# lyclyc52/Segment-Anything-NeRF

Measured on AMD Instinct MI355X. Metric: rays/sec (RGB+256-d SAM feat) at 512×512, 1/2/4/8 MI355X; PSNR vs ref, higher is better.
Workload: dtype fp32-equivalent: fp32 in the reference's op order for everything that decides a discrete result (near/far, bins, proposal grids + MLPs, compositing, sample_pdf); grid_mlp (32->64->64->16 per sample), the SAM head (163->256x5) and the mask head (143->256->256->K per sample) as f16x3: each fp32 produc

## Files before the change

### segment-anything-nerf_amd/csrc/sam_head.hip

```cpp
#include "samnerf_common.h"
#include "f16x3.h"

namespace samnerf {

namespace {

constexpr int kRows = 32;
constexpr int kXPad = 168;
constexpr int kXStride = 169;
constexpr int kHStride = 257;
constexpr int kIn = 163;
constexpr int kRowIn = 164;
constexpr int kK[5] = {kXPad, 256, 256 + kXPad, 256, 256};
constexpr int kGroups[5] = {kXPad / 8, 256 / 8, (256 + kXPad) / 8, 256 / 8, 256 / 8};
constexpr int kLogicalIn[5] = {kIn, 256, 256 + kIn, 256, 256};

__host__ __device__ constexpr int group_base(int layer) {
    int b = 0;
    for (int i = 0; i < layer; ++i) b += kGroups[i];
    return b;
}
constexpr int kTotalGroups = group_base(5);

__device__ __forceinline__ int logical_k(int layer, int kp) {
// ... 596 lines not shown
    const char* rows;
    const char* rows_end;
    uint32_t xs;
    uint32_t next_tile;
    int wave, lane;
    int rot;
    int step;

    __device__ __forceinline__ int buf(int s) const {
        const int b = rot + s % NBUF;
        return b >= NBUF ? b - NBUF : b;
    }
    __device__ __forceinline__ void wpiece(int s, int c) {
        const uint4* base = packed + (size_t)(s % kSteps) * kStepVec + (size_t)wave * 256 + (size_t)c * 64;
        lds_dma16(base + lane, (uint32_t)reinterpret_cast<uintptr_t>(Wb + buf(s) * kStepVec + wave * 256 + c * 64));
    }
    __device__ __forceinline__ void xpiece(int q) {
        const uint32_t p = (uint32_t)(wave * kXPieces + q);
        const char* base = rows + (size_t)next_tile * kTileBytes + (size_t)p * 1024u;
        const char* src = base + (size_t)lane * 16u;
        src = src > rows_end ? rows_end : src;
        lds_dma16(src, xs + p * 1024u);
    }
    static __device__ __forceinline__ constexpr bool xstep(int s) { return s >= kXFirst && s < kXFirst + kXPieces; }

    __device__ __forceinline__ void run(floatx16 (&acc)[8], const uint4& bh, const uint4& bl) {
        const int s = step;
        const uint4* cur = Wb + buf(s) * kStepVec + lane;
        uint4 fh[8], fl[8];
#pragma unroll
        for (int t = 0; t < 8; ++t) {
            fh[t] = cur[t * 64];
            fl[t] = cur[512 + t * 64];
        }
#pragma unroll
        for (int t = 0; t < 8; ++t) {
            acc[t] = mfma_f16x3(fh[t], fl[t], bh, bl, acc[t]);
            if (t & 1) {
                __builtin_amdgcn_sched_barrier(0);
                wpiece(s + NBUF - 1, t >> 1);
                __builtin_amdgcn_sched_barrier(0);
            }
        }
        if (xstep(s)) {
            __builtin_amdgcn_sched_barrier(0);
            xpiece(s - kXFirst);
            __builtin_amdgcn_sched_barrier(0);
        }
        int n = 4 * (NBUF - 2);
#pragma unroll
        for (int k = s + 2 - NBUF; k <= s; ++k) n += xstep(k) ? 1 : 0;
        wait_vmn(n);
        asm volatile("s_waitcnt lgkmcnt(0)" ::: "memory");
        __builtin_amdgcn_s_barrier();
        ++step;
    }
};

template <int NBUF, bool STAMP = false, bool VEC = true>
__global__ void __launch_bounds__(256) __attribute__((amdgpu_waves_per_eu(1, 1)))
k_sam_head_h16q(HeadArgsH a, uint32_t ntiles) {
    unsigned long long t0 = 0, rt0 = 0;
    if constexpr (STAMP) {
        t0 = __builtin_amdgcn_s_memtime();
        rt0 = __builtin_amdgcn_s_memrealtime();
    }
    __shared__ uint4 smem[NBUF * kStepVec + kXVec + (7 * 256 + 8) / 4];
    uint4* const Wb = smem;
    float* const Xs = reinterpret_cast<float*>(smem + NBUF * kStepVec);
    float* const Bs = reinterpret_cast<float*>(smem + NBUF * kStepVec + kXVec);
    const int tid = threadIdx.x, wave = tid >> 6, lane = tid & 63;
    const int j = lane & 31, h = lane >> 5;

    for (int i = tid; i < 5 * 256; i += 256) Bs[i] = a.b[i >> 8][i & 255];
    float* const Wi = Bs + 7 * 256;
    if (tid < 5) Wi[tid] = exp2i(-a.kexp[tid]);
    Bs[5 * 256 + tid] = a.ln_w[tid];
    Bs[6 * 256 + tid] = a.ln_b[tid];

    HeadStreamQ<NBUF> st;
    st.packed = a.packed + (size_t)((blockIdx.x >> 3) % kHeadCopies) * kPackedVec;
    st.Wb = Wb;
    st.rows = reinterpret_cast<const char*>(a.rows);
    st.rows_end = st.rows + (size_t)a.N * kRowIn * 4 - 16;
    st.xs = (uint32_t)reinterpret_cast<uintptr_t>(Xs);
    st.next_tile = blockIdx.x;
    st.wave = __builtin_amdgcn_readfirstlane(wave);
    st.lane = lane;
    st.rot = 0;
    st.step = 0;
#pragma unroll
    for (int q = 0; q < kXPieces; ++q) st.xpiece(q);
#pragma unroll
    for (int q = 0; q + 1 < NBUF; ++q)
#pragma unroll
        for (int c = 0; c < 4; ++c) st.wpiece(q, c);
    wait_vmn(4 * (NBUF - 2));
    asm volatile("s_waitcnt lgkmcnt(0)" ::: "memory");
    __syncthreads();

    const float* xr = Xs + (wave * 32 + j) * kRowIn;
    for (uint32_t tile = blockIdx.x; tile < ntiles; tile += gridDim.x) {
        st.next_tile = tile + gridDim.x;
        st.step = 0;
        asm volatile("" : "+s"(st.packed), "+s"(st.rows));
        const uint32_t ray = tile * kRaysV5 + wave * 32u + j;
        const bool live = ray < a.N;
        auto x8 = [&](int kb, float (&v)[8]) {
            const int c0 = 16 * kb + 8 * h;
            if (c0 + 8 <= kRowIn) {
                const float4 p = *reinterpret_cast<const float4*>(xr + c0);
                const float4 q = *reinterpret_cast<const float4*>(xr + c0 + 4);
                v[0] = p.x; v[1] = p.y; v[2] = p.z; v[3] = p.w;
                v[4] = q.x; v[5] = q.y; v[6] = q.z; v[7] = q.w;
            } else {
#pragma unroll
                for (int m = 0; m < 8; ++m) v[m] = c0 + m < kRowIn ? xr[c0 + m] : 0.0f;
            }
#pragma unroll
            for (int m = 0; m < 8; ++m)
                if (!live || c0 + m >= kIn) v[m] = 0.0f;
        };
        float xmax = 0.0f;
#pragma unroll
        for (int kb = 0; kb < kXkb; ++kb) {
            float v[8];
            x8(kb, v);
#pragma unroll
            for (int m = 0; m < 8; ++m) xmax = fmaxf(xmax, fabsf(v[m]));
        }
        xmax = fmaxf(xmax, __shfl_xor(xmax, 32));
        auto load_x = [&](float sc_s, uint4 (&xh)[kXkb], uint4 (&xl)[kXkb]) {
#pragma unroll
            for (int kb = 0; kb < kXkb; ++kb) {
                float v[8];
                x8(kb, v);
                split8_f16(v, sc_s, xh[kb], xl[kb]);
            }
        };
        uint4 xh[kXkb], xl[kXkb];
        Scale2 sc = scale_of_max(xmax);
        load_x(sc.s, xh, xl);

        floatx16 acc[8];
        uint4 ah[kHkb], al[kHkb];
        auto zero = [&]() {
#pragma unroll
            for (int t = 0; t < 8; ++t) acc[t] = floatx16{};
        };
        auto next = [&](int layer, float extra) {
            float m = finish_layer(acc, Bs + layer * 256, sc.inv * Wi[layer], h, true);
            m = fmaxf(fmaxf(m, __shfl_xor(m, 32)), extra);
            sc = scale_of_max(m);
            split_layer(acc, sc.s, ah, al);
        };
        auto h_segment = [&]() {
#pragma unroll
            for (int kb = 0; kb < kHkb; ++kb) st.run(acc, ah[kb], al[kb]);
        };

        zero();
#pragma unroll
        for (int kb = 0; kb < kXkb; ++kb) st.run(acc, xh[kb], xl[kb]);
        next(0, 0.0f);
        zero();
        h_segment();
        next(1, xmax);
        zero();
        load_x(sc.s, xh, xl);
#pragma unroll
        for (int kb = 0; kb < kXkb; ++kb) st.run(acc, xh[kb], xl[kb]);
        h_segment();
        next(2, 0.0f);
        zero();
        h_segment();
        next(3, 0.0f);
        zero();
        h_segment();
        finish_layer(acc, Bs + 4 * 256, sc.inv * Wi[4], h, false);

        double s = 0.0;
#pragma unroll
        for (int t = 0; t < 8; ++t)
#pragma unroll
            for (int q = 0; q < 16; ++q) s += (double)acc[t][q];
        s += __shfl_xor(s, 32);
        const double mean = s / 256.0;
        double var = 0.0;
#pragma unroll
        for (int t = 0; t < 8; ++t)
#pragma unroll
            for (int q = 0; q < 16; ++q) {
                const double dlt = (double)acc[t][q] - mean;
                var += dlt * dlt;
            }
        var += __shfl_xor(var, 32);
        const float rstd = (float)(1.0 / sqrt(var / 256.0 + 1e-5));
        const float mf = (float)mean;
        if (live) {
            float* o = a.out + (size_t)ray * a.ld;
            const float* lw = Bs + 5 * 256;
            const float* lb = Bs + 6 * 256;
#pragma unroll
            for (int t = 0; t < 8; ++t)
#pragma unroll
                for (int mm = 0; mm < 4; ++mm) {
                    const int u = 32 * t + 8 * mm + 4 * h;
                    float4 y;
                    y.x = ((acc[t][4 * mm + 0] - mf) * rstd) * lw[u + 0] + lb[u + 0];
                    y.y = ((acc[t][4 * mm + 1] - mf) * rstd) * lw[u + 1] + lb[u + 1];
                    y.z = ((acc[t][4 * mm + 2] - mf) * rstd) * lw[u + 2] + lb[u + 2];
                    y.w = ((acc[t][4 * mm + 3] - mf) * rstd) * lw[u + 3] + lb[u + 3];
                    store_out4(o + u, y, VEC);
                }
        }
        st.rot = (st.rot + kSteps) % NBUF;
    }
    wait_vmn(0);
    if constexpr (STAMP) {
        const unsigned long long t1 = __builtin_amdgcn_s_memtime(), rt1 = __builtin_amdgcn_s_memrealtime();
        if (lane == 0) {
            unsigned long long* o = a.stamps + ((size_t)blockIdx.x * 4 + wave) * 16;
            for (int i = 0; i < 16; ++i) o[i] = 0;
            o[12] = t1 - t0;
            o[13] = rt1 - rt0;
        }
    }
}

#ifndef SAMNERF_HEAD_W8
#define SAMNERF_HEAD_W8 1
#endif
#if defined(SAMNERF_DIAG_VARIANTS) || SAMNERF_HEAD_W8
namespace w8 {
constexpr int kXkb = 6;
constexpr int kHkb = 8;
constexpr int kSegKb[6] = {kXkb, kHkb, kXkb, kHkb, kHkb, kHkb};
constexpr int kSegLayer[6] = {0, 1, 2, 2, 3, 4};
constexpr int segBase(int seg) {
    int b = 0;
    for (int i = 0; i < seg; ++i) b += kSegKb[i];
    return b;
}
constexpr int kKb = segBase(6);
constexpr int kSteps = 2 * kKb;
constexpr int kStepVec = 2 * 8 * 64;
constexpr int kPackedVec = kSteps * kStepVec;
constexpr int kRays = 16;
constexpr int kWaves = 8;
constexpr int kXPieces = 11;
constexpr int kXRegion = 84;
constexpr int kXFirst = 30;
static_assert(kXPieces * kWaves * 1024 >= kTileBytes, "x pieces cover a tile");
static_assert(kXRegion * 1024 >= kTileBytes && kXRegion * 1024 <= kXVec * 16, "x region");
static_assert(kXFirst > 2 * (kXkb + kHkb) + 1 && kXFirst + kXPieces + 3 < kSteps, "x stream window");

__host__ __device__ constexpr int hunit(int b, int g, int m) { return 32 * b + (m < 4 ? 4 * g + m : 16 + 4 * g + m - 4); }

__device__ __forceinline__ float weight(const float* const* W, int kb, int unit, int g, int m) {
    int seg = 0;
    while (seg < 5 && kb >= segBase(seg + 1)) ++seg;
    const int b = kb - segBase(seg);
    const int kx = 32 * b + 8 * g + m;
    switch (seg) {
        case 0: return kx < kIn ? W[0][unit * kIn + kx] : 0.0f;
        case 1: return W[1][unit * 256 + hunit(b, g, m)];
        case 2: return kx < kIn ? W[2][unit * (256 + kIn) + 256 + kx] : 0.0f;
        case 3: return W[2][unit * (256 + kIn) + hunit(b, g, m)];
        case 4: return W[3][unit * 256 + hunit(b, g, m)];
        default: return W[4][unit * 256 + hunit(b, g, m)];
    }
}
}

__global__ void __launch_bounds__(256) k_pack_w8(PackArgs a) {
    __shared__ int kx;
    const uint32_t t = blockIdx.x * blockDim.x + threadIdx.x;
    const int bstep = (int)((blockIdx.x * blockDim.x) >> 9);
    int bseg = 0;
    while (bseg < 5 && (bstep >> 1) >= w8::segBase(bseg + 1)) ++bseg;
    const int layer = w8::kSegLayer[bseg];
    if (threadIdx.x < 64) {
        float m = threadIdx.x < kWmaxParts ? a.part[layer * kWmaxParts + threadIdx.x] : 0.0f;
        m = wave_max64(m);
        if (threadIdx.x == 0) {
            kx = scale_exp_of_max(m);
            a.kexp[layer] = kx;
        }
    }
    __syncthreads();
    if (t >= (uint32_t)w8::kSteps * 8u * 64u) return;
    const int lane = (int)(t & 63u), tile = (int)((t >> 6) & 7u), step = (int)(t >> 9);
    const int kb = step >> 1, unit = 16 * (8 * (step & 1) + tile) + (lane & 15), g = lane >> 4;
    float v[8];
#pragma unroll
    for (int e = 0; e < 8; ++e) v[e] = w8::weight(a.W, kb, unit, g, e);
    uint4 hi, lo;
    split8_f16(v, exp2i(kx), hi, lo);
    a.packed[(size_t)step * w8::kStepVec + tile * 64 + lane] = hi;
    a.packed[(size_t)step * w8::kStepVec + 512 + tile * 64 + lane] = lo;
}


template <int NBUF, int WAVES>
struct HeadStreamW8 {
    static constexpr int kPieces = 16 / WAVES;
    const uint4* packed;
    uint4* Wb;
    const char* rows;
    const char* rows_end;
    uint32_t xs;
    uint32_t sink;
    uint32_t next_tile;
    int wave, lane;
    int rot;
    int step;

    __device__ __forceinline__ int buf(int s) const {
        const int b = rot + s % NBUF;
        return b >= NBUF ? b - NBUF : b;
    }
    __device__ __forceinline__ void wpiece(int s, int c) {
        const int o = wave * 64 * kPieces + c * 64;
        const uint4* base = packed + (size_t)(s % w8::kSteps) * w8::kStepVec + (size_t)o;
        lds_dma16(base + lane, (uint32_t)reinterpret_cast<uintptr_t>(Wb + buf(s) * w8::kStepVec + o));
    }
    __device__ __forceinline__ void xpiece(int q) {
        const uint32_t p = (uint32_t)(wave * w8::kXPieces + q);
        const char* src = rows + (size_t)next_tile * kTileBytes + (size_t)p * 1024u + (size_t)lane * 16u;
        src = src > rows_end ? rows_end : src;
        lds_dma16(src, p < (uint32_t)w8::kXRegion ? xs + p * 1024u : sink);
    }
    static __device__ __forceinline__ constexpr bool xstep(int s) {
        return WAVES == 8 && s >= w8::kXFirst && s < w8::kXFirst + w8::kXPieces;
    }

    template <int HALF>
    __device__ __forceinline__ void run(floatx4 (&acc)[16], const uint4& bh, const uint4& bl) {
        const int s = step;
        const uint4* cur = Wb + buf(s) * w8::kStepVec + lane;
        uint4 fh[8], fl[8];
#pragma unroll
        for (int t = 0; t < 8; ++t) {
            fh[t] = cur[t * 64];
            fl[t] = cur[512 + t * 64];
        }
#pragma unroll
        for (int t = 0; t < 8; ++t) {
            acc[8 * HALF + t] = mfma16_f16x3(fh[t], fl[t], bh, bl, acc[8 * HALF + t]);
            if (t % (8 / kPieces) == 8 / kPieces - 1) {
                __builtin_amdgcn_sched_barrier(0);
                wpiece(s + NBUF - 1, t / (8 / kPieces));
                __builtin_amdgcn_sched_barrier(0);
            }
        }
        if (xstep(s)) {
            __builtin_amdgcn_sched_barrier(0);
            xpiece(s - w8::kXFirst);
            __builtin_amdgcn_sched_barrier(0);
        }
        int n = kPieces * (NBUF - 2);
#pragma unroll
        for (int k = s + 2 - NBUF; k <= s; ++k) n += xstep(k) ? 1 : 0;
        wait_vmn(n);
        asm volatile("s_waitcnt lgkmcnt(0)" ::: "memory");
        __builtin_amdgcn_s_barrier();
        ++step;
    }
};

__device__ __forceinline__ float finish_w8(floatx4 (&acc)[16], const float* Bs, float inv, int g, bool act) {
    float m = 0.0f;
#pragma unroll
    for (int t = 0; t < 16; ++t) {
        const float4 bb = *reinterpret_cast<const float4*>(Bs + 16 * t + 4 * g);
        const float b4[4] = {bb.x, bb.y, bb.z, bb.w};
#pragma unroll
        for (int r = 0; r < 4; ++r) acc[t][r] = leaky(__builtin_fmaf(acc[t][r], inv, b4[r]), act);
        m = max_abs3(m, acc[t][0], acc[t][1]);
        m = max_abs3(m, acc[t][2], acc[t][3]);
    }
    return m;
}

__device__ __forceinline__ void split_w8(const floatx4 (&acc)[16], float s, uint4 (&ah)[w8::kHkb],
                                         uint4 (&al)[w8::kHkb]) {
#pragma unroll
    for (int b = 0; b < w8::kHkb; ++b) {
        const float v[8] = {acc[2 * b][0], acc[2 * b][1], acc[2 * b][2], acc[2 * b][3],
                            acc[2 * b + 1][0], acc[2 * b + 1][1], acc[2 * b + 1][2], acc[2 * b + 1][3]};
        split8_f16<true>(v, s, ah[b], al[b]);
    }
}

__device__ __forceinline__ float ray_max4(float m) {
    m = fmaxf(m, __shfl_xor(m, 16));
    return fmaxf(m, __shfl_xor(m, 32));
}
__device__ __forceinline__ double ray_sum4(double v) {
    v += __shfl_xor(v, 16);
    return v + __shfl_xor(v, 32);
}

constexpr int kW8SinkVec = 64;

template <int NBUF, int WAVES, bool VEC = true>
__global__ void __launch_bounds__(64 * WAVES) __attribute__((amdgpu_waves_per_eu(2, 2)))
k_sam_head_w8(HeadArgsH a, uint32_t ntiles) {
    constexpr bool XLDS = WAVES == 8;
    constexpr int kTileRays = WAVES * w8::kRays;
    constexpr int kX = XLDS ? kXVec + kW8SinkVec : 0;
    __shared__ uint4 smem[NBUF * w8::kStepVec + kX + (7 * 256 + 8) / 4];
    uint4* const Wb = smem;
    float* const Xs = reinterpret_cast<float*>(smem + NBUF * w8::kStepVec);
    float* const Bs = reinterpret_cast<float*>(smem + NBUF * w8::kStepVec + kX);
    const int tid = threadIdx.x, wave = tid >> 6, lane = tid & 63;
    const int j = lane & 15, g = lane >> 4;
    if (XLDS && wave >= 4) __builtin_amdgcn_s_setprio(1);

    for (int i = tid; i < 5 * 256; i += 64 * WAVES) Bs[i] = a.b[i >> 8][i & 255];
    float* const Wi = Bs + 7 * 256;
    if (tid < 5) Wi[tid] = exp2i(-a.kexp[tid]);
    if (tid < 256) {
        Bs[5 * 256 + tid] = a.ln_w[tid];
        Bs[6 * 256 + tid] = a.ln_b[tid];
    }

    HeadStreamW8<NBUF, WAVES> st;
    st.packed = a.packed;
    st.Wb = Wb;
    st.rows = reinterpret_cast<const char*>(a.rows);
    st.rows_end = st.rows + (size_t)a.N * kRowIn * 4 - 16;
    st.xs = (uint32_t)reinterpret_cast<uintptr_t>(Xs);
    st.sink = (uint32_t)reinterpret_cast<uintptr_t>(smem + NBUF * w8::kStepVec + kXVec);
    st.next_tile = blockIdx.x;
    st.wave = __builtin_amdgcn_readfirstlane(wave);
    st.lane = lane;
    st.rot = 0;
    st.step = 0;
    if constexpr (XLDS) {
#pragma unroll
        for (int q = 0; q < w8::kXPieces; ++q) st.xpiece(q);
    }
#pragma unroll
    for (int q = 0; q + 1 < NBUF; ++q)
#pragma unroll
        for (int c = 0; c < st.kPieces; ++c) st.wpiece(q, c);
    wait_vmn(st.kPieces * (NBUF - 2));
    asm volatile("s_waitcnt lgkmcnt(0)" ::: "memory");
    __syncthreads();

    for (uint32_t tile = blockIdx.x; tile < ntiles; tile += gridDim.x) {
        st.next_tile = tile + gridDim.x;
        st.step = 0;
        asm volatile("" : "+s"(st.packed), "+s"(st.rows));
        const uint32_t ray = tile * kTileRays + wave * w8::kRays + j;
        const bool live = ray < a.N;
        const float* xr = XLDS ? Xs + (wave * w8::kRays + j) * kRowIn : a.rows + (size_t)(live ? ray : 0u) * kRowIn;
        auto x8 = [&](int kb, float (&v)[8]) {
            const int c0 = 32 * kb + 8 * g;
            if (c0 + 8 <= kRowIn) {
                const float4 p = *reinterpret_cast<const float4*>(xr + c0);
                const float4 q = *reinterpret_cast<const float4*>(xr + c0 + 4);
                v[0] = p.x; v[1] = p.y; v[2] = p.z; v[3] = p.w;
                v[4] = q.x; v[5] = q.y; v[6] = q.z; v[7] = q.w;
            } else {
#pragma unroll
                for (int m = 0; m < 8; ++m) v[m] = c0 + m < kRowIn ? xr[c0 + m] : 0.0f;
            }
#pragma unroll
            for (int m = 0; m < 8; ++m)
                if (!live || c0 + m >= kIn) v[m] = 0.0f;
        };
        float xmax = 0.0f;
#pragma unroll
        for (int kb = 0; kb < w8::kXkb; ++kb) {
            float v[8];
            x8(kb, v);
#pragma unroll
            for (int m = 0; m < 8; ++m) xmax = fmaxf(xmax, fabsf(v[m]));
        }
        xmax = ray_max4(xmax);
        uint4 xh[w8::kXkb], xl[w8::kXkb];
        auto load_x = [&](float sc_s) {
#pragma unroll
            for (int kb = 0; kb < w8::kXkb; ++kb) {
                float v[8];
                x8(kb, v);
                split8_f16<true>(v, sc_s, xh[kb], xl[kb]);
            }
        };
        Scale2 sc = scale_of_max(xmax);
        load_x(sc.s);

        floatx4 acc[16];
        uint4 ah[w8::kHkb], al[w8::kHkb];
        auto zero = [&]() {
#pragma unroll
            for (int t = 0; t < 16; ++t) acc[t] = floatx4{};
        };
        auto next = [&](int layer, float extra) {
            float m = finish_w8(acc, Bs + layer * 256, sc.inv * Wi[layer], g, true);
            m = fmaxf(ray_max4(m), extra);
            sc = scale_of_max(m);
            split_w8(acc, sc.s, ah, al);
        };
        auto x_segment = [&]() {
#pragma unroll
            for (int kb = 0; kb < w8::kXkb; ++kb) {
                st.template run<0>(acc, xh[kb], xl[kb]);
                st.template run<1>(acc, xh[kb], xl[kb]);
            }
        };
        auto h_segment = [&]() {
#pragma unroll
            for (int kb = 0; kb < w8::kHkb; ++kb) {
                st.template run<0>(acc, ah[kb], al[kb]);
                st.template run<1>(acc, ah[kb], al[kb]);
            }
        };

        zero();
        x_segment();
        next(0, 0.0f);
        zero();
        h_segment();
        next(1, xmax);
        zero();
        load_x(sc.s);
        x_segment();
        h_segment();
        next(2, 0.0f);
        zero();
        h_segment();
        next(3, 0.0f);
        zero();
        h_segment();
        finish_w8(acc, Bs + 4 * 256, sc.inv * Wi[4], g, false);

        double s = 0.0;
#pragma unroll
        for (int t = 0; t < 16; ++t)
#pragma unroll
            for (int r = 0; r < 4; ++r) s += (double)acc[t][r];
        s = ray_sum4(s);
        const double mean = s / 256.0;
        double var = 0.0;
#pragma unroll
        for (int t = 0; t < 16; ++t)
#pragma unroll
            for (int r = 0; r < 4; ++r) {
                const double dlt = (double)acc[t][r] - mean;
                var += dlt * dlt;
            }
        var = ray_sum4(var);
        const float rstd = (float)(1.0 / sqrt(var / 256.0 + 1e-5));
        const float mf = (float)mean;
        if (live) {
            float* o = a.out + (size_t)ray * a.ld;
            const float* lw = Bs + 5 * 256;
            const float* lb = Bs + 6 * 256;
#pragma unroll
            for (int t = 0; t < 16; ++t) {
                const int u = 16 * t + 4 * g;
                float4 y;
                y.x = ((acc[t][0] - mf) * rstd) * lw[u + 0] + lb[u + 0];
                y.y = ((acc[t][1] - mf) * rstd) * lw[u + 1] + lb[u + 1];
                y.z = ((acc[t][2] - mf) * rstd) * lw[u + 2] + lb[u + 2];
                y.w = ((acc[t][3] - mf) * rstd) * lw[u + 3] + lb[u + 3];
                store_out4(o + u, y, VEC);
            }
        }
        st.rot = (st.rot + w8::kSteps) % NBUF;
    }
    wait_vmn(0);
}
#endif

#ifdef SAMNERF_DIAG_VARIANTS
template <int TPW>
struct PairCfg {
    static constexpr int WPG = 8 / TPW;
    static constexpr int NW = 4 * WPG;
    static constexpr int NT = 64 * NW;
    static constexpr int PIECES = 16 / NW;
};
constexpr int kBVec = kHkb * 2 * 64;
constexpr int kPairSmemVec = 2 * kStepVec + 4 * kBVec;

__device__ __forceinline__ void lds_barrier() {
    asm volatile("s_waitcnt lgkmcnt(0)" ::: "memory");
    __builtin_amdgcn_s_barrier();
    asm volatile("" ::: "memory");
}

template <int TPW>
__global__ void __launch_bounds__(PairCfg<TPW>::NT)
__attribute__((amdgpu_waves_per_eu(PairCfg<TPW>::WPG, PairCfg<TPW>::WPG)))
k_sam_head_h16p(HeadArgsH a) {
    using C = PairCfg<TPW>;
    __shared__ uint4 smem[kPairSmemVec];
    uint4* const Wb = smem;
    const int tid = threadIdx.x, wave = tid >> 6, lane = tid & 63;
    const int grp = wave / C::WPG, part = wave % C::WPG;
    const int t0 = part * TPW;
    uint4* const Bg = smem + 2 * kStepVec + grp * kBVec;
    const int j = lane & 31, h = lane >> 5;
    const uint32_t ray = blockIdx.x * kRaysV5 + grp * 32u + j;
    const bool live = ray < a.N;
    const float* xr = a.rows + (size_t)(live ? ray : 0u) * kRowIn;

    auto issue = [&](int s) {
        const uint4* src = a.packed + (size_t)s * kStepVec + wave * (64 * C::PIECES) + lane;
        const uint32_t dst = (uint32_t)reinterpret_cast<uintptr_t>(Wb + (s & 1) * kStepVec + wave * (64 * C::PIECES));
#pragma unroll
        for (int c = 0; c < C::PIECES; ++c) lds_dma16(src + c * 64, dst + c * 1024u);
    };
    auto xload = [&](int kb, float4& p, float4& q) {
        if (kb < kXkb - 1) {
            p = *reinterpret_cast<const float4*>(xr + 16 * kb + 8 * h);
            q = *reinterpret_cast<const float4*>(xr + 16 * kb + 8 * h + 4);
        } else {
            p = *reinterpret_cast<const float4*>(xr + 160);
            q = p;
        }
    };
    auto xvals = [&](int kb, const float4& p, const float4& q, float (&v)[8]) {
        v[0] = p.x; v[1] = p.y; v[2] = p.z; v[3] = p.w;
        v[4] = q.x; v[5] = q.y; v[6] = q.z; v[7] = q.w;
        const int c0 = 16 * kb + 8 * h;
#pragma unroll
        for (int m = 0; m < 8; ++m)
            if (!live || c0 + m >= kIn) v[m] = 0.0f;
    };

    int s = 0;
    issue(0);
    float xmax = 0.0f;
#pragma unroll
    for (int kb = 0; kb < kXkb; ++kb) {
        float4 p, q;
        float v[8];
        xload(kb, p, q);
        xvals(kb, p, q, v);
#pragma unroll
        for (int m = 0; m < 8; ++m) xmax = fmaxf(xmax, fabsf(v[m]));
    }
    xmax = fmaxf(xmax, __shfl_xor(xmax, 32));
    float Wi[5];
#pragma unroll
    for (int l = 0; l < 5; ++l) Wi[l] = exp2i(-a.kexp[l]);
    Scale2 sc = scale_of_max(xmax);
    asm volatile("s_waitcnt vmcnt(0)" ::: "memory");
    lds_barrier();

    floatx16 acc[TPW];
    auto zero = [&]() {
#pragma unroll
        for (int t = 0; t < TPW; ++t) acc[t] = floatx16{};
    };
    auto mma = [&](const uint4& bh, const uint4& bl) {
        const uint4* cur = Wb + (s & 1) * kStepVec + lane;
        uint4 fh[TPW], fl[TPW];
#pragma unroll
        for (int t = 0; t < TPW; ++t) {
            fh[t] = cur[(t0 + t) * 64];
            fl[t] = cur[512 + (t0 + t) * 64];
        }
#pragma unroll
        for (int t = 0; t < TPW; ++t) acc[t] = mfma_f16x3(fh[t], fl[t], bh, bl, acc[t]);
        asm volatile("s_waitcnt vmcnt(0)" ::: "memory");
        lds_barrier();
        ++s;
    };
    auto x_segment = [&]() {
        float4 p, q;
        xload(0, p, q);
#pragma unroll
        for (int kb = 0; kb < kXkb; ++kb) {
            float v[8];
            xvals(kb, p, q, v);
            uint4 bh, bl;
            split8_f16(v, sc.s, bh, bl);
            if (s + 1 < kSteps) issue(s + 1);
            if (kb + 1 < kXkb) xload(kb + 1, p, q);
            mma(bh, bl);
        }
    };
    auto h_segment = [&]() {
#pragma unroll
        for (int kb = 0; kb < kHkb; ++kb) {
            const uint4 bh = Bg[(2 * kb) * 64 + lane], bl = Bg[(2 * kb + 1) * 64 + lane];
            if (s + 1 < kSteps) issue(s + 1);
            mma(bh, bl);
        }
    };
    auto next = [&](int layer, float extra) {
        const float inv = sc.inv * Wi[layer];
        const float* bias = a.b[layer];
        float m = 0.0f;
#pragma unroll
        for (int t = 0; t < TPW; ++t)
#pragma unroll
            for (int mm = 0; mm < 4; ++mm) {
                const float4 bb = *reinterpret_cast<const float4*>(bias + 32 * (t0 + t) + 8 * mm + 4 * h);
                const float b4[4] = {bb.x, bb.y, bb.z, bb.w};
#pragma unroll
                for (int e = 0; e < 4; ++e)
                    acc[t][4 * mm + e] = leaky(__builtin_fmaf(acc[t][4 * mm + e], inv, b4[e]), true);
#pragma unroll
                for (int e = 0; e < 4; e += 2) m = max_abs3(m, acc[t][4 * mm + e], acc[t][4 * mm + e + 1]);
            }
        m = fmaxf(m, __shfl_xor(m, 32));
        float* X = reinterpret_cast<float*>(Wb + ((s + 1) & 1) * kStepVec);
        if (h == 0) X[(grp * C::WPG + part) * 32 + j] = m;
        lds_barrier();
        float mm2 = 0.0f;
#pragma unroll
        for (int p = 0; p < C::WPG; ++p) mm2 = fmaxf(mm2, X[(grp * C::WPG + p) * 32 + j]);
        sc = scale_of_max(fmaxf(mm2, extra));
#pragma unroll
        for (int t = 0; t < TPW; ++t) {
            float v[16];
#pragma unroll
            for (int q = 0; q < 16; ++q) v[q] = acc[t][q];
            uint4 hi, lo;
            split8_f16(v, sc.s, hi, lo);
            Bg[(2 * (2 * (t0 + t))) * 64 + lane] = hi;
            Bg[(2 * (2 * (t0 + t)) + 1) * 64 + lane] = lo;
            split8_f16(v + 8, sc.s, hi, lo);
            Bg[(2 * (2 * (t0 + t) + 1)) * 64 + lane] = hi;
            Bg[(2 * (2 * (t0 + t) + 1) + 1) * 64 + lane] = lo;
        }
        lds_barrier();
    };

    zero();
    x_segment();
    next(0, 0.0f);
    zero();
    h_segment();
    next(1, xmax);
    zero();
    x_segment();
    h_segment();
    next(2, 0.0f);
    zero();
    h_segment();
    next(3, 0.0f);
    zero();
    h_segment();

    float4* Y = reinterpret_cast<float4*>(Bg);
    {
        const float inv = sc.inv * Wi[4];
        const float* bias = a.b[4];
#pragma unroll
        for (int t = 0; t < TPW; ++t)
#pragma unroll
            for (int mm = 0; mm < 4; ++mm) {
                const float4 bb = *reinterpret_cast<const float4*>(bias + 32 * (t0 + t) + 8 * mm + 4 * h);
                float4 y;
                y.x = __builtin_fmaf(acc[t][4 * mm + 0], inv, bb.x);
                y.y = __builtin_fmaf(acc[t][4 * mm + 1], inv, bb.y);
                y.z = __builtin_fmaf(acc[t][4 * mm + 2], inv, bb.z);
                y.w = __builtin_fmaf(acc[t][4 * mm + 3], inv, bb.w);
                Y[((t0 + t) * 4 + mm) * 64 + lane] = y;
            }
    }
    lds_barrier();
    double sum = 0.0;
#pragma unroll
    for (int t = 0; t < 8; ++t) {
#pragma unroll
        for (int mm = 0; mm < 4; ++mm) {
            const float4 y = Y[(t * 4 + mm) * 64 + lane];
            sum += (double)y.x;
            sum += (double)y.y;
            sum += (double)y.z;
            sum += (double)y.w;
        }
        asm volatile("" ::: "memory");
    }
    sum += __shfl_xor(sum, 32);
    const double mean = sum / 256.0;
    double var = 0.0;
#pragma unroll
    for (int t = 0; t < 8; ++t) {
#pragma unroll
        for (int mm = 0; mm < 4; ++mm) {
            const float4 y = Y[(t * 4 + mm) * 64 + lane];
            const float yy[4] = {y.x, y.y, y.z, y.w};
#pragma unroll
            for (int e = 0; e < 4; ++e) {
                const double dlt = (double)yy[e] - mean;
                var += dlt * dlt;
            }
        }
        asm volatile("" ::: "memory");
    }
    var += __shfl_xor(var, 32);
    const float rstd = (float)(1.0 / sqrt(var / 256.0 + 1e-5));
    const float mf = (float)mean;
    if (!live) return;
    float* o = a.out + (size_t)ray * a.ld;
#pragma unroll
    for (int t = 0; t < TPW; ++t)
#pragma unroll
        for (int mm = 0; mm < 4; ++mm) {
            const int u = 32 * (t0 + t) + 8 * mm + 4 * h;
            const float4 v = Y[((t0 + t) * 4 + mm) * 64 + lane];
            const float4 lw = *reinterpret_cast<const float4*>(a.ln_w + u);
            const float4 lb = *reinterpret_cast<const float4*>(a.ln_b + u);
            float4 y;
            y.x = ((v.x - mf) * rstd) * lw.x + lb.x;
            y.y = ((v.y - mf) * rstd) * lw.y + lb.y;
            y.z = ((v.z - mf) * rstd) * lw.z + lb.z;
            y.w = ((v.w - mf) * rstd) * lw.w + lb.w;
            store_out4(o + u, y, a.vec_out);
        }
}

#endif

}

static int device_cus() {
    static int cus[64] = {0};
    int dev = 0;
    if (hipGetDevice(&dev) != hipSuccess || dev < 0 || dev >= 64) return 256;
    if (!cus[dev]) {
        int n = 0;
        if (hipDeviceGetAttribute(&n, hipDeviceAttributeMultiprocessorCount, dev) != hipSuccess || n <= 0) n = 256;
        cus[dev] = n;
    }
    return cus[dev];
}

[[maybe_unused]] static int head_w8() {
#ifdef SAMNERF_DIAG_VARIANTS
    const char* v = diag_env("SAMNERF_HEAD_V");
    if (v) return atoi(v) == 30 ? 1 : atoi(v) == 31 ? 2 : 0;
#endif
    return SAMNERF_HEAD_W8;
}

size_t sam_head_packed_floats() {
    const size_t f32 = (size_t)8 * kTotalGroups * 64 * 4;
    const size_t h16 = (size_t)kPackedVec * 4 * kHeadCopies + 8 + 5 * kWmaxParts;
    const size_t hw8 = (size_t)88 * 1024 * 4 + 8 + 5 * kWmaxParts;
    const size_t m = f32 > h16 ? f32 : h16;
    return m > hw8 ? m : hw8;
}

int sam_head_forward(const samnerf_model* m, const float* rows, uint32_t N, float* samvit,
                     float* packed, hipStream_t s, uint32_t ld, bool pack) {
    const bool vec = ld % 4u == 0u && reinterpret_cast<uintptr_t>(samvit) % 16u == 0u;
#if defined(SAMNERF_DIAG_VARIANTS) || SAMNERF_HEAD_W8
    if (m->head_mode == 0 && head_w8()) {
        PackArgs p;
        for (int i = 0; i < 5; ++i) p.W[i] = m->sam_w[i];
        p.packed = reinterpret_cast<uint4*>(packed);
        p.kexp = reinterpret_cast<int*>(packed + (size_t)w8::kPackedVec * 4);
        p.part = packed + (size_t)w8::kPackedVec * 4 + 8;
        if (pack) {
            k_head_wmax<<<dim3(kWmaxParts, 5), 256, 0, s>>>(p);
            k_pack_w8<<<div_up((uint32_t)w8::kSteps * 8u * 64u, 256), 256, 0, s>>>(p);
        }
        HeadArgsH a{};
        a.rows = rows;
        a.N = N;
        a.packed = p.packed;
        a.kexp = p.kexp;
        for (int i = 0; i < 5; ++i) a.b[i] = m->sam_b[i];
        a.ln_w = m->ln_w;
        a.ln_b = m->ln_b;
        a.out = samvit;
        a.ld = ld;
        a.vec_out = vec;
        if (head_w8() == 2) {
            const uint32_t blocks = div_up(N, 64u);
            const uint32_t grid = blocks < 2u * (uint32_t)device_cus() ? blocks : 2u * (uint32_t)device_cus();
            if (vec) k_sam_head_w8<4, 4><<<grid, 256, 0, s>>>(a, blocks);
            else k_sam_head_w8<4, 4, false><<<grid, 256, 0, s>>>(a, blocks);
        } else {
            const uint32_t blocks = div_up(N, (uint32_t)kRaysV5);
            const uint32_t grid = blocks < (uint32_t)device_cus() ? blocks : (uint32_t)device_cus();
            if (vec) k_sam_head_w8<4, 8><<<grid, 512, 0, s>>>(a, blocks);
            else k_sam_head_w8<4, 8, false><<<grid, 512, 0, s>>>(a, blocks);
        }
        return check_launch("sam_head_w8");
    }
#endif
    if (m->head_mode == 0) {
        PackArgs p;
        for (int i = 0; i < 5; ++i) p.W[i] = m->sam_w[i];
        p.packed = reinterpret_cast<uint4*>(packed);
        p.kexp = reinterpret_cast<int*>(packed + (size_t)kPackedVec * 4 * kHeadCopies);
        p.part = packed + (size_t)kPackedVec * 4 * kHeadCopies + 8;
        if (pack) {
            k_head_wmax<<<dim3(kWmaxParts, 5), 256, 0, s>>>(p);
            k_pack_h16<<<div_up((uint32_t)kSteps * 8u * 64u, 256), 256, 0, s>>>(p);
        }
        HeadArgsH a;
        a.rows = rows;
        a.N = N;
        a.packed = p.packed;
        a.kexp = p.kexp;
        for (int i = 0; i < 5; ++i) a.b[i] = m->sam_b[i];
        a.ln_w = m->ln_w;
        a.ln_b = m->ln_b;
        a.out = samvit;
        a.ld = ld;
        a.vec_out = vec;
        a.stamps = nullptr;
        const uint32_t blocks = div_up(N, (uint32_t)kRaysV5);
#ifdef SAMNERF_DIAG_VARIANTS
        const char* v = diag_env("SAMNERF_HEAD_V");
        const int form = v ? atoi(v) : 0;
        const uint32_t grid = blocks < (uint32_t)device_cus() ? blocks : (uint32_t)device_cus();
        if (form == 20) k_sam_head_h16q<3><<<grid, 256, 0, s>>>(a, blocks);
        else if (form == 21 || form == 13) {
            const char* p = diag_env("SAMNERF_HEAD_STAMPS");
            a.stamps = reinterpret_cast<unsigned long long*>(p ? strtoull(p, nullptr, 16) : 0ull);
            if (!a.stamps) return fail(SAMNERF_EINVAL, "sam_head form %d needs SAMNERF_HEAD_STAMPS", form);
            if (form == 21) k_sam_head_h16q<4, true><<<grid, 256, 0, s>>>(a, blocks);
            else k_sam_head_h16<3, true, 1, false, true><<<blocks, 256, 0, s>>>(a);
        }
        else if (form == 1) k_sam_head_h16<3, false, 1><<<blocks, 256, 0, s>>>(a);
        else if (form == 2) k_sam_head_h16p<4><<<blocks, PairCfg<4>::NT, 0, s>>>(a);
        else if (form == 3) k_sam_head_h16p<2><<<blocks, PairCfg<2>::NT, 0, s>>>(a);
        else if (form == 5) k_sam_head_h16<3, false, 2><<<blocks, 256, 0, s>>>(a);
        else if (form == 6) k_sam_head_h16<4, true, 1><<<blocks, 256, 0, s>>>(a);
        else if (form == 7) k_sam_head_h16<3, true, 2><<<blocks, 256, 0, s>>>(a);
        else if (form == 8) k_sam_head_h16<4, true, 2><<<blocks, 256, 0, s>>>(a);
        else if (form == 11) k_sam_head_h16<3, true, 0><<<blocks, 256, 0, s>>>(a);
        else if (form == 12) k_sam_head_h16<3, true, 1, true><<<blocks, 256, 0, s>>>(a);
        else if (form == 4) k_sam_head_h16<3, true, 1><<<blocks, 256, 0, s>>>(a);
        else
#endif
        {
            const uint32_t grid = blocks < (uint32_t)device_cus() ? blocks : (uint32_t)device_cus();
            if (vec) k_sam_head_h16q<4><<<grid, 256, 0, s>>>(a, blocks);
            else k_sam_head_h16q<4, false, false><<<grid, 256, 0, s>>>(a, blocks);
        }
        return check_launch("sam_head_h16");
    }
    const uint32_t nvec = 8u * kTotalGroups * 64u;
    if (pack)
        k_pack<<<div_up(nvec, 256), 256, 0, s>>>(m->sam_w[0], m->sam_w[1], m->sam_w[2], m->sam_w[3],
                                                 m->sam_w[4], packed);
    HeadArgs a;
    a.rows = rows;
    a.N = N;
    a.packed = packed;
    for (int i = 0; i < 5; ++i) a.b[i] = m->sam_b[i];
    a.ln_w = m->ln_w;
    a.ln_b = m->ln_b;
    a.out = samvit;
    a.ld = ld;
    a.vec_out = vec;
    k_sam_head<<<div_up(N, kRows), 256, 0, s>>>(a);
    return check_launch("sam_head");
}

}

extern "C" {

size_t samnerf_sam_head_workspace_size(void) { return samnerf::sam_head_packed_floats() * sizeof(float); }

int samnerf_sam_head_forward(const samnerf_model* m, const float* rows, uint32_t N, float* samvit,
                             void* workspace, size_t workspace_bytes, samnerf_stream_t stream) {
    using namespace samnerf;
    if (!m) return fail(SAMNERF_EINVAL, "sam_head_forward: null model");
    if (!m->with_sam) return fail(SAMNERF_EINVAL, "sam_head_forward: model has no SAM head (with_sam = 0)");
    for (int i = 0; i < 5; ++i)
        if (!m->sam_w[i] || !m->sam_b[i]) return fail(SAMNERF_EINVAL, "sam_head_forward: null head weight");
    if (!m->ln_w || !m->ln_b) return fail(SAMNERF_EINVAL, "sam_head_forward: null LayerNorm weight");
    if (m->head_mode != 0 && m->head_mode != 1)
        return fail(SAMNERF_EINVAL, "sam_head_forward: head_mode must be 0 or 1, got %d", m->head_mode);
    if (N == 0) return SAMNERF_OK;
    if (!rows || !samvit || !workspace) return fail(SAMNERF_EINVAL, "sam_head_forward: null pointer");
    const size_t need = samnerf_sam_head_workspace_size();
    if (workspace_bytes < need)
        return fail(SAMNERF_EWORKSPACE, "sam_head_forward: workspace needs %zu bytes, got %zu", need,
                    workspace_bytes);
    return sam_head_forward(m, rows, N, samvit, static_cast<float*>(workspace),
                            reinterpret_cast<hipStream_t>(stream), 256u, true);
}

}
```

Before: 98.29 million.

## Software-pipeline LDS weight fragment loads across steps in the W8 SAM head

Adds a pipelined loop for the 8-wave W8 SAM head kernel. Half of the next step's weight fragments are read from LDS before the barrier while the current MFMAs run, and the DMA of the next weight piece now runs one step further ahead using all NBUF buffers. The default path now uses the pipelined variant with both pieces issued at the last MFMA (PLACE=1). It also adds diagnostic variants with timestamp probes, and an output-address tweak that uses mbcnt for the lane group. The aim is to hide LDS read latency and barrier stalls behind MFMA work, at the cost of more register pressure from holding fragments in the struct and tighter buffer reuse.

```diff
diff --git a/segment-anything-nerf_amd/csrc/sam_head.hip b/segment-anything-nerf_amd/csrc/sam_head.hip
--- a/segment-anything-nerf_amd/csrc/sam_head.hip
+++ b/segment-anything-nerf_amd/csrc/sam_head.hip
@@ -922,9 +922,12 @@
 }
 
 
-template <int NBUF, int WAVES>
+template <int NBUF, int WAVES, bool PIPE = false, bool STAMP = false, int PLACE = 0>
 struct HeadStreamW8 {
     static constexpr int kPieces = 16 / WAVES;
+    static constexpr int kAhead = PIPE ? NBUF : NBUF - 1;
+    uint4 fh[8], fl[8];
+    unsigned long long ts[4];
     const uint4* packed;
     uint4* Wb;
     const char* rows;
@@ -940,8 +943,10 @@
         const int b = rot + s % NBUF;
         return b >= NBUF ? b - NBUF : b;
     }
+    static constexpr bool kLowMoves = PLACE == 2;
+    __device__ __forceinline__ bool mover() const { return !kLowMoves || wave < 4; }
     __device__ __forceinline__ void wpiece(int s, int c) {
-        const int o = wave * 64 * kPieces + c * 64;
+        const int o = wave * 64 * (kLowMoves ? 4 : kPieces) + c * 64;
         const uint4* base = packed + (size_t)(s % w8::kSteps) * w8::kStepVec + (size_t)o;
         lds_dma16(base + lane, (uint32_t)reinterpret_cast<uintptr_t>(Wb + buf(s) * w8::kStepVec + o));
     }
@@ -955,16 +960,28 @@
         return WAVES == 8 && s >= w8::kXFirst && s < w8::kXFirst + w8::kXPieces;
     }
 
+    static __device__ __forceinline__ unsigned long long now() {
+        unsigned long long t = __builtin_amdgcn_s_memtime();
+        asm volatile("s_waitcnt lgkmcnt(0)" : "+s"(t)::"memory");
+        return t;
+    }
+
     template <int HALF>
     __device__ __forceinline__ void run(floatx4 (&acc)[16], const uint4& bh, const uint4& bl) {
+        if constexpr (PIPE) {
+            run_pipe<HALF>(acc, bh, bl);
+            return;
+        }
         const int s = step;
         const uint4* cur = Wb + buf(s) * w8::kStepVec + lane;
-        uint4 fh[8], fl[8];
+        unsigned long long t0 = 0, t1 = 0, t2 = 0;
+        if constexpr (STAMP) t0 = now();
 #pragma unroll
         for (int t = 0; t < 8; ++t) {
             fh[t] = cur[t * 64];
             fl[t] = cur[512 + t * 64];
         }
+        if constexpr (STAMP) t1 = now();
 #pragma unroll
         for (int t = 0; t < 8; ++t) {
             acc[8 * HALF + t] = mfma16_f16x3(fh[t], fl[t], bh, bl, acc[8 * HALF + t]);
@@ -979,13 +996,94 @@
             xpiece(s - w8::kXFirst);
             __builtin_amdgcn_sched_barrier(0);
         }
+        if constexpr (STAMP) t2 = now();
         int n = kPieces * (NBUF - 2);
 #pragma unroll
         for (int k = s + 2 - NBUF; k <= s; ++k) n += xstep(k) ? 1 : 0;
         wait_vmn(n);
         asm volatile("s_waitcnt lgkmcnt(0)" ::: "memory");
         __builtin_amdgcn_s_barrier();
+        if constexpr (STAMP) {
+            const unsigned long long t3 = now();
+            ts[0] += t1 - t0;
+            ts[1] += t2 - t1;
+            ts[2] += t3 - t2;
+        }
         ++step;
+    }
+
+    template <int HALF>
+    __device__ __forceinline__ void run_pipe(floatx4 (&acc)[16], const uint4& bh, const uint4& bl) {
+        const int s = step;
+        const uint4* cur = Wb + buf(s) * w8::kStepVec + lane;
+        const uint4* nxt = Wb + buf(s + 1) * w8::kStepVec + lane;
+        unsigned long long t0 = 0, t1 = 0, t2 = 0;
+        if constexpr (STAMP) t0 = now();
+#pragma unroll
+        for (int t = 4; t < 8; ++t) {
+            fh[t] = cur[t * 64];
+            fl[t] = cur[512 + t * 64];
+        }
+        __builtin_amdgcn_sched_barrier(0);
+#pragma unroll
+        for (int t = 0; t < 4; ++t) acc[8 * HALF + t] = mfma16_f16x3(fh[t], fl[t], bh, bl, acc[8 * HALF + t]);
+        __builtin_amdgcn_sched_barrier(0);
+        if constexpr (STAMP) t1 = now();
+        int n = 0;
+#pragma unroll
+        for (int k = s + 1 - NBUF; k < s; ++k) n += xstep(k) ? 1 : 0;
+        if constexpr (kLowMoves) {
+            if (wave < 4) wait_vmn(n + 4 * (NBUF - 2));
+            else wait_vmn(n);
+        } else {
+            wait_vmn(n + kPieces * (NBUF - 2));
+        }
+        asm volatile("s_waitcnt lgkmcnt(0)" ::: "memory");
+        __builtin_amdgcn_s_barrier();
+        if constexpr (STAMP) t2 = now();
+#pragma unroll
+        for (int t = 0; t < 4; ++t) {
+            fh[t] = nxt[t * 64];
+            fl[t] = nxt[512 + t * 64];
+        }
+        __builtin_amdgcn_sched_barrier(0);
+#pragma unroll
+        for (int t = 4; t < 8; ++t) {
+            acc[8 * HALF + t] = mfma16_f16x3(fh[t], fl[t], bh, bl, acc[8 * HALF + t]);
+            if (PLACE == 0 ? (t & 1) : t == 7) {
+                __builtin_amdgcn_sched_barrier(0);
+                if (PLACE == 0) wpiece(s + NBUF, (t - 4) >> 1);
+                else if (PLACE == 1) {
+                    wpiece(s + NBUF, 0);
+                    wpiece(s + NBUF, 1);
+                } else if (wave < 4) {
+#pragma unroll
+                    for (int c = 0; c < 4; ++c) wpiece(s + NBUF, c);
+                }
+                __builtin_amdgcn_sched_barrier(0);
+            }
+        }
+        if (xstep(s)) {
+            __builtin_amdgcn_sched_barrier(0);
+            xpiece(s - w8::kXFirst);
+            __builtin_amdgcn_sched_barrier(0);
+        }
+        if constexpr (STAMP) {
+            const unsigned long long t3 = now();
+            ts[0] += t1 - t0;
+            ts[1] += t2 - t1;
+            ts[2] += t3 - t2;
+        }
+        ++step;
+    }
+
+    __device__ __forceinline__ void prime() {
+        const uint4* cur = Wb + buf(0) * w8::kStepVec + lane;
+#pragma unroll
+        for (int t = 0; t < 4; ++t) {
+            fh[t] = cur[t * 64];
+            fl[t] = cur[512 + t * 64];
+        }
     }
 };
 
@@ -1024,9 +1122,10 @@
 
 constexpr int kW8SinkVec = 64;
 
-template <int NBUF, int WAVES, bool VEC = true>
+template <int NBUF, int WAVES, bool VEC = true, bool PIPE = false, bool STAMP = false, int PLACE = 0>
 __global__ void __launch_bounds__(64 * WAVES) __attribute__((amdgpu_waves_per_eu(2, 2)))
 k_sam_head_w8(HeadArgsH a, uint32_t ntiles) {
+    static_assert(!PIPE || WAVES == 8, "the pipelined loop places two pieces per wave and step");
     constexpr bool XLDS = WAVES == 8;
     constexpr int kTileRays = WAVES * w8::kRays;
     constexpr int kX = XLDS ? kXVec + kW8SinkVec : 0;
@@ -1046,7 +1145,7 @@
         Bs[6 * 256 + tid] = a.ln_b[tid];
     }
 
-    HeadStreamW8<NBUF, WAVES> st;
+    HeadStreamW8<NBUF, WAVES, PIPE, STAMP, PLACE> st;
     st.packed = a.packed;
     st.Wb = Wb;
     st.rows = reinterpret_cast<const char*>(a.rows);
@@ -1062,17 +1161,25 @@
 #pragma unroll
         for (int q = 0; q < w8::kXPieces; ++q) st.xpiece(q);
     }
-#pragma unroll
-    for (int q = 0; q + 1 < NBUF; ++q)
-#pragma unroll
-        for (int c = 0; c < st.kPieces; ++c) st.wpiece(q, c);
-    wait_vmn(st.kPieces * (NBUF - 2));
+    if (st.mover()) {
+#pragma unroll
+        for (int q = 0; q < st.kAhead; ++q)
+#pragma unroll
+            for (int c = 0; c < (st.kLowMoves ? 4 : st.kPieces); ++c) st.wpiece(q, c);
+        wait_vmn((st.kLowMoves ? 4 : st.kPieces) * (NBUF - 2));
+    } else {
+        wait_vmn(0);
+    }
     asm volatile("s_waitcnt lgkmcnt(0)" ::: "memory");
     __syncthreads();
+    if constexpr (PIPE) st.prime();
 
     for (uint32_t tile = blockIdx.x; tile < ntiles; tile += gridDim.x) {
         st.next_tile = tile + gridDim.x;
         st.step = 0;
+        if constexpr (STAMP) st.ts[0] = st.ts[1] = st.ts[2] = st.ts[3] = 0;
+        unsigned long long tile_t0 = 0;
+        if constexpr (STAMP) tile_t0 = st.now();
         asm volatile("" : "+s"(st.packed), "+s"(st.rows));
         const uint32_t ray = tile * kTileRays + wave * w8::kRays + j;
         const bool live = ray < a.N;
@@ -1177,21 +1284,33 @@
         const float rstd = (float)(1.0 / sqrt(var / 256.0 + 1e-5));
         const float mf = (float)mean;
         if (live) {
-            float* o = a.out + (size_t)ray * a.ld;
-            const float* lw = Bs + 5 * 256;
-            const float* lb = Bs + 6 * 256;
+            int ln;
+            asm volatile("v_mbcnt_lo_u32_b32 %0, -1, 0\n\tv_mbcnt_hi_u32_b32 %0, -1, %0" : "=v"(ln));
+            const int g4 = 4 * (ln >> 4);
+            float* o = a.out + (size_t)ray * a.ld + g4;
+            const float* lw = Bs + 5 * 256 + g4;
+            const float* lb = Bs + 6 * 256 + g4;
 #pragma unroll
             for (int t = 0; t < 16; ++t) {
-                const int u = 16 * t + 4 * g;
                 float4 y;
-                y.x = ((acc[t][0] - mf) * rstd) * lw[u + 0] + lb[u + 0];
-                y.y = ((acc[t][1] - mf) * rstd) * lw[u + 1] + lb[u + 1];
-                y.z = ((acc[t][2] - mf) * rstd) * lw[u + 2] + lb[u + 2];
-                y.w = ((acc[t][3] - mf) * rstd) * lw[u + 3] + lb[u + 3];
-                store_out4(o + u, y, VEC);
+                y.x = ((acc[t][0] - mf) * rstd) * lw[16 * t + 0] + lb[16 * t + 0];
+                y.y = ((acc[t][1] - mf) * rstd) * lw[16 * t + 1] + lb[16 * t + 1];
+                y.z = ((acc[t][2] - mf) * rstd) * lw[16 * t + 2] + lb[16 * t + 2];
+                y.w = ((acc[t][3] - mf) * rstd) * lw[16 * t + 3] + lb[16 * t + 3];
+                store_out4(o + 16 * t, y, VEC);
             }
         }
         st.rot = (st.rot + w8::kSteps) % NBUF;
+        if constexpr (STAMP) {
+            const uint32_t it = (tile - blockIdx.x) / gridDim.x;
+            if (blockIdx.x == 0 && it < 4 && lane == 0) {
+                unsigned long long* o = a.stamps + ((size_t)it * WAVES + wave) * 4;
+                o[0] = st.ts[0];
+                o[1] = st.ts[1];
+                o[2] = st.ts[2];
+                o[3] = st.now() - tile_t0;
+            }
+        }
     }
     wait_vmn(0);
 }
@@ -1460,7 +1579,10 @@
 [[maybe_unused]] static int head_w8() {
 #ifdef SAMNERF_DIAG_VARIANTS
     const char* v = diag_env("SAMNERF_HEAD_V");
-    if (v) return atoi(v) == 30 ? 1 : atoi(v) == 31 ? 2 : 0;
+    if (v) {
+        const int f = atoi(v);
+        return f == 30 ? 1 : f == 31 ? 2 : f >= 32 && f <= 37 ? f - 29 : 0;
+    }
 #endif
     return SAMNERF_HEAD_W8;
 }
@@ -1506,8 +1628,34 @@
         } else {
             const uint32_t blocks = div_up(N, (uint32_t)kRaysV5);
             const uint32_t grid = blocks < (uint32_t)device_cus() ? blocks : (uint32_t)device_cus();
-            if (vec) k_sam_head_w8<4, 8><<<grid, 512, 0, s>>>(a, blocks);
-            else k_sam_head_w8<4, 8, false><<<grid, 512, 0, s>>>(a, blocks);
+#ifdef SAMNERF_DIAG_VARIANTS
+            if (head_w8() == 3) {
+                if (vec) k_sam_head_w8<4, 8><<<grid, 512, 0, s>>>(a, blocks);
+                else k_sam_head_w8<4, 8, false><<<grid, 512, 0, s>>>(a, blocks);
+                return check_launch("sam_head_w8");
+            }
+            if (head_w8() == 6) {
+                if (vec) k_sam_head_w8<4, 8, true, true, false, 2><<<grid, 512, 0, s>>>(a, blocks);
+                else k_sam_head_w8<4, 8, false, true, false, 2><<<grid, 512, 0, s>>>(a, blocks);
+                return check_launch("sam_head_w8");
+            }
+            if (head_w8() == 8) {
+                if (vec) k_sam_head_w8<4, 8, true, true, false, 0><<<grid, 512, 0, s>>>(a, blocks);
+                else k_sam_head_w8<4, 8, false, true, false, 0><<<grid, 512, 0, s>>>(a, blocks);
+                return check_launch("sam_head_w8");
+            }
+            if (head_w8() >= 4) {
+                const char* sp = diag_env("SAMNERF_HEAD_STAMPS");
+                a.stamps = reinterpret_cast<unsigned long long*>(sp ? strtoull(sp, nullptr, 16) : 0ull);
+                if (!a.stamps) return fail(SAMNERF_EINVAL, "sam_head forms 33 / 34 / 36 need SAMNERF_HEAD_STAMPS");
+                if (head_w8() == 4) k_sam_head_w8<4, 8, true, false, true><<<grid, 512, 0, s>>>(a, blocks);
+                else if (head_w8() == 5) k_sam_head_w8<4, 8, true, true, true, 1><<<grid, 512, 0, s>>>(a, blocks);
+                else k_sam_head_w8<4, 8, true, true, true, 2><<<grid, 512, 0, s>>>(a, blocks);
+                return check_launch("sam_head_w8");
+            }
+#endif
+            if (vec) k_sam_head_w8<4, 8, true, true, false, 1><<<grid, 512, 0, s>>>(a, blocks);
+            else k_sam_head_w8<4, 8, false, true, false, 1><<<grid, 512, 0, s>>>(a, blocks);
         }
         return check_launch("sam_head_w8");
     }
```

After: 99.10 million (median of 6 runs). Within noise of the previous version (+0.8%).
